# Leo-Liao-Chao/Uncertainty-Aware-CILQR-for-Trajectory-Optimization

Measured on AMD Instinct MI355X. Metric: CILQR solves/sec (N=50, batch B), higher is better.
Workload: dtype f64

## Files before the change

### uncertainty-aware-cilqr-for-trajectory-optimization_amd/csrc/cilqr_api.cpp

```cpp
#include <math.h>
#include <stdarg.h>
#include <stdio.h>
#include <stdlib.h>
#include <string.h>

#include <new>
#include <string>

#include "cilqr_internal.h"

#include "cilqr_handle.h"

namespace cilqr {
thread_local std::string g_last_error;

int fail(int code, const char* fmt, ...) {
  char buf[512];
  va_list ap;
  va_start(ap, fmt);
  vsnprintf(buf, sizeof(buf), fmt, ap);
  va_end(ap);
  g_last_error = buf;
  return code;
}
// ... 166 lines not shown

  cilqr_handle* h = new (std::nothrow) cilqr_handle();
  if (!h) return fail(CILQR_ERR_ARG, "out of host memory");
  memset(h, 0, sizeof(*h));
  h->params = *p;
  derive(*p, h->kp);
  h->device = device;
  h->simds = prop.multiProcessorCount > 0 ? prop.multiProcessorCount * 4 : 1024;
  h->max_batch = max_batch; h->max_horizon = max_horizon; h->max_obstacles = max_obstacles;
  if (const char* fg = getenv("CILQR_FORCE_G")) h->force_g = atoi(fg);
  const size_t B = max_batch, N = max_horizon, M = max_obstacles;
  hipError_t err = hipStreamCreateWithFlags(&h->stream, hipStreamNonBlocking);
  {
    const cilqr::IoLayout plain = cilqr::io_layout(B, N, M, true, 0), sampled = cilqr::io_layout(B, N, M, false, 1);
    h->arena_cap = plain.end > sampled.end ? plain.end : sampled.end;
    if (err == hipSuccess) err = hipMalloc((void**)&h->d_arena, h->arena_cap);
    h->stage_cap = h->arena_cap < ((size_t)1 << 20) ? h->arena_cap : ((size_t)1 << 20);
    if (err == hipSuccess) err = hipHostMalloc((void**)&h->stage, h->stage_cap, hipHostMallocDefault);
  }
  const size_t Bpad = (B + 63) / 64 * 64;
  if (err == hipSuccess) err = dmalloc(&h->d_obs_tab, Bpad * M * N * 6);
  if (err == hipSuccess) err = dmalloc(&h->d_ws, cilqr::solve_groups_ws_doubles(max_batch, max_horizon));
  if (err == hipSuccess) err = dmalloc(&h->d_redo, B);
  if (err == hipSuccess) err = dmalloc(&h->d_hint_passes, B);
  if (err == hipSuccess) err = dmalloc(&h->d_order, B);
  h->hint_B = 0; h->hint_stream = nullptr;
  h->hint_off = getenv("CILQR_NO_SCHEDULE_HINT") != nullptr;
  h->pair_on = getenv("CILQR_PAIR_KERNEL") != nullptr;
  h->steal_off = getenv("CILQR_NO_LANE_SHARING") != nullptr;
  h->split_off = getenv("CILQR_NO_SPLIT_KERNEL") != nullptr;
  h->share_off = getenv("CILQR_NO_SHARE_KERNEL") != nullptr;
  if (const char* kb = getenv("CILQR_LDS_TABLE_KB")) h->tab_budget_kb = atoi(kb);
  h->share_max = -1;
  if (const char* sw = getenv("CILQR_SHARE_W")) h->share_w = atoi(sw) == 3 ? 3 : 2;
  if (const char* sm = getenv("CILQR_SHARE_MAX_B")) h->share_max = atoi(sm);
  if (const char* sw = getenv("CILQR_SPLIT_W")) h->split_w = atoi(sw);
  if (err == hipSuccess) err = dmalloc(&h->d_pair, (size_t)2);
  if (err == hipSuccess) err = dmalloc(&h->d_triple, (size_t)3);
  if (err == hipSuccess) err = dmalloc(&h->d_gather, (size_t)3);
  h->comm_ranks = 1;
  if (err == hipSuccess) err = dmalloc(&h->d_oob, (size_t)1);
  if (err == hipSuccess) err = dmalloc(&h->d_poses, (size_t)8 * 1024 * 4);
  if (err == hipSuccess) err = dmalloc(&h->d_occ_steps, (size_t)8 * 128);
  if (err == hipSuccess) {
    void* unused = nullptr;
    const size_t W = (size_t)p->num_of_local_wpts;
    if (cilqr::scratch_bytes(h, cilqr::SCR_PLAN_IO, (B * (4 + CILQR_POLY_COEFFS + 2 + 2 * W)) * sizeof(double) + B * sizeof(int32_t), &unused) != CILQR_OK ||
        cilqr::scratch_bytes(h, cilqr::SCR_PLAN_PATH, 2 * 1024 * sizeof(double), &unused) != CILQR_OK)
      err = hipErrorOutOfMemory;
  }
  if (err != hipSuccess) {
    int rc = fail(CILQR_ERR_HIP, "cilqr_create: device allocation failed: %s", hipGetErrorString(err));
    cilqr_destroy(h);
    return rc;
  }
  *out = h;
  return CILQR_OK;
}

int cilqr_destroy(cilqr_handle* h) {
  if (!h) return CILQR_OK;
  (void)hipSetDevice(h->device);
  if (h->stream) (void)hipStreamSynchronize(h->stream);
  (void)cilqr_comm_destroy(h);
  if (h->stage) (void)hipHostFree(h->stage);
  for (void* p : h->scratch)
    if (p) (void)hipFree(p);
  void* ptrs[] = {h->d_poses, h->d_unc_layer, h->d_triple, h->d_gather, h->d_arena, h->d_obs_tab, h->d_ws, h->d_redo, h->d_hint_passes, h->d_order, h->d_pair, h->d_src, h->d_dst, h->d_bbox, h->d_oob, h->d_occ_steps};
  for (void* p : ptrs)
    if (p) (void)hipFree(p);
  if (h->stream) (void)hipStreamDestroy(h->stream);
  delete h;
  return CILQR_OK;
}

int cilqr_set_diag_buffer(cilqr_handle* h, uint64_t* dev_buf) {
  if (!h) return fail(CILQR_ERR_ARG, "null handle");
  h->diag = (unsigned long long*)dev_buf;
  return CILQR_OK;
}

namespace {
int fill_unc(const cilqr_handle* h, const cilqr_uncertainty_map* m, cilqr::UncArgs& u) {
  if (!m || !m->layer) return fail(CILQR_ERR_ARG, "cilqr_set_uncertainty_map: null map or layer");
  const cilqr_map_geom& g = m->geom;
  if (g.rows < 2 || g.cols < 2 || !(g.res > 0.0) || !(g.len_x > 0.0) || !(g.len_y > 0.0))
    return fail(CILQR_ERR_ARG, "cilqr_set_uncertainty_map: bad geometry (needs at least 2x2 cells)");
  if (m->probes_l < 1 || m->probes_w < 1 || m->probes_l > 64 || m->probes_w > 64)
    return fail(CILQR_ERR_ARG, "cilqr_set_uncertainty_map: probes_l / probes_w must be in [1, 64]");
  if (m->layer_stride < 0 || (m->layer_stride > 0 && m->layer_stride < (int64_t)g.rows * g.cols))
    return fail(CILQR_ERR_ARG, "cilqr_set_uncertainty_map: layer_stride smaller than one layer");
// ... 146 lines not shown
  const int w = pick_split_wavefronts(h, B);
  if (w < 2 || N > 64 || n_obs < w) return 1;
  return w >= 4 ? 4 : 2;
}

int cilqr_solve_batch_device(cilqr_handle* h, void* stream, int B, int N, int M, const double* x0, double* U,
                             const double* poly, const double* xplan_fl, const double* obs_pose, const double* obs_dim,
                             const double* obs_weight, double* X_out, double* J_out, int32_t* iters_out,
                             int32_t* status_out, uint32_t flags) {
  int rc = check_sizes(h, B, N, M);
  if (rc) return rc;
  if (B == 0) return CILQR_OK;
  if (!x0 || !U || !poly || !xplan_fl || !X_out) return fail(CILQR_ERR_ARG, "cilqr_solve_batch: null required pointer");
  if (M > 0 && (!obs_pose || !obs_dim)) return fail(CILQR_ERR_ARG, "cilqr_solve_batch: M > 0 but obstacle tables are null");
  cilqr::SolveArgs a;
  a.x0 = x0; a.U = U; a.poly = poly; a.xplan_fl = xplan_fl;
  a.obs_pose = obs_pose; a.obs_dim = obs_dim; a.obs_weight = M > 0 ? obs_weight : nullptr;
  a.X_out = X_out; a.J_out = J_out; a.iters_out = iters_out; a.status_out = status_out;
  a.samp_off = nullptr; a.n_samples = 0; a.samp_w = 0.0;
  a.obs_tab = h->d_obs_tab;
  a.fwd = h->d_ws;
  a.order = nullptr; a.hint_passes = nullptr; a.pair = 0; a.tab_budget = 0; a.steal = h->steal_off ? 0 : 1; a.split = 0;
  a.redo = h->d_redo;
  a.diag = h->diag;
  a.passes = h->passes;
  a.unc = h->unc;
  a.B = B; a.N = N; a.M = M; a.flags = flags;
  a.kp = h->kp;
  HIP_TRY(hipSetDevice(h->device));
  const int G = pick_group_lanes(h, B, N, M);
  if (G == 64 && cilqr::solve_lds_bytes(N, h->kp.n_samples) > cilqr::SOLVE_LDS_MAX)
    return fail(CILQR_ERR_UNSUPPORTED, "cilqr_solve_batch: horizon %d needs %zu bytes of LDS per solve (limit %zu)", N,
                cilqr::solve_lds_bytes(N, h->kp.n_samples), cilqr::SOLVE_LDS_MAX);
  if (G == 64) return launch_wave_scheduled(h, a, stream);
  HIP_TRY(cilqr::launch_solve_groups(a, G, h->d_ws, (hipStream_t)stream));
  return CILQR_OK;
}

}

extern "C" {

int cilqr_solve_batch(cilqr_handle* h, int B, int N, int M, const double* x0, double* U, const double* poly,
                      const double* xplan_fl, const double* obs_pose, const double* obs_dim, const double* obs_weight,
                      double* X_out, double* J_out, int32_t* iters_out, int32_t* status_out, uint32_t flags) {
  int rc = check_sizes(h, B, N, M);
// ... 12 lines not shown
                                     const double* nom_dim, const double* sample_offset, double sample_weight, double* X_out,
                                     double* J_out, int32_t* iters_out, int32_t* status_out, uint32_t flags) {
  if (n_obs < 1 || n_samples < 2) return fail(CILQR_ERR_ARG, "cilqr_solve_batch_sampled: needs n_obs >= 1 and n_samples >= 2");
  if ((long)n_obs * n_samples > 1 << 20) return fail(CILQR_ERR_ARG, "cilqr_solve_batch_sampled: n_obs * n_samples too large");
  int rc = check_sizes(h, B, N, n_obs * n_samples);
  if (rc) return rc;
  if (B == 0) return CILQR_OK;
  if (!x0 || !U || !poly || !xplan_fl || !X_out || !nom_pose || !nom_dim || !sample_offset)
    return fail(CILQR_ERR_ARG, "cilqr_solve_batch_sampled: null required pointer");
  if (cilqr::solve_lds_bytes(N, h->kp.n_samples) + cilqr::solve_sampled_lds_bytes(n_obs, n_samples) > cilqr::SOLVE_LDS_MAX)
    return fail(CILQR_ERR_UNSUPPORTED, "cilqr_solve_batch_sampled: n_obs * n_samples offset records do not fit LDS beside the solve");
  if (cilqr::solve_sampled_tab_doubles(n_obs, N) > (size_t)h->max_obstacles * 6 * (size_t)h->max_horizon)
    return fail(CILQR_ERR_UNSUPPORTED, "cilqr_solve_batch_sampled: nominal records exceed the obstacle workspace reserved at create");
  cilqr::SolveArgs a;
  a.x0 = x0; a.U = U; a.poly = poly; a.xplan_fl = xplan_fl;
  a.obs_pose = nom_pose; a.obs_dim = nom_dim; a.obs_weight = nullptr;
  a.X_out = X_out; a.J_out = J_out; a.iters_out = iters_out; a.status_out = status_out;
  a.samp_off = sample_offset; a.n_samples = n_samples; a.samp_w = sample_weight;
  a.obs_tab = h->d_obs_tab;
  a.fwd = h->d_ws;
  a.pair = 0; a.tab_budget = 0; a.steal = 0;
  a.split = pick_split_wavefronts(h, B);
  a.redo = h->d_redo;
  a.diag = h->diag;
  a.passes = h->passes;
  a.unc = h->unc;
  a.B = B; a.N = N; a.M = n_obs; a.flags = flags;
  a.kp = h->kp;
  HIP_TRY(hipSetDevice(h->device));
  return launch_wave_scheduled(h, a, stream);
}

int cilqr_solve_batch_sampled(cilqr_handle* h, int B, int N, int n_obs, int n_samples, const double* x0, double* U,
                              const double* poly, const double* xplan_fl, const double* nom_pose, const double* nom_dim,
                              const double* sample_offset, double sample_weight, double* X_out, double* J_out,
                              int32_t* iters_out, int32_t* status_out, uint32_t flags) {
  if (n_obs < 1 || n_samples < 2) return fail(CILQR_ERR_ARG, "cilqr_solve_batch_sampled: needs n_obs >= 1 and n_samples >= 2");
  if ((long)n_obs * n_samples > 1 << 20) return fail(CILQR_ERR_ARG, "cilqr_solve_batch_sampled: n_obs * n_samples too large");
  int rc = check_sizes(h, B, N, n_obs * n_samples);
  if (rc) return rc;
  if (B == 0) return CILQR_OK;
  if (!x0 || !U || !poly || !xplan_fl || !X_out || !nom_pose || !nom_dim || !sample_offset)
    return fail(CILQR_ERR_ARG, "cilqr_solve_batch_sampled: null required pointer");
  cilqr::HostBatch q{B, N, n_obs, n_samples, x0, U, poly, xplan_fl, nom_pose, nom_dim, nullptr, sample_offset, sample_weight, X_out, J_out,
                     iters_out, status_out, flags};
  rc = cilqr::host_solve_enqueue(h, q);
// ... 287 lines not shown
```

### uncertainty-aware-cilqr-for-trajectory-optimization_amd/csrc/cilqr_handle.h

```cpp
#pragma once

#include <string>

#include "cilqr_internal.h"

struct ncclComm;

struct cilqr_handle;

namespace cilqr {
struct IoLayout {
  size_t x0, poly, xplan, obs_w, samp_off, obs_pose, obs_dim, U, X, J, iters, status, end;
};
IoLayout io_layout(size_t B, size_t N, size_t M, bool weights, size_t n_samples);
struct HostBatch {
  int B, N, M, n_samples;
  const double *x0;
  double* U;
  const double *poly, *xplan_fl, *obs_pose, *obs_dim, *obs_weight, *samp_off;
  double samp_w;
  double *X_out, *J_out;
  int32_t *iters_out, *status_out;
  uint32_t flags;
};
// ... 16 lines not shown
    hipError_t e_ = (expr);                                                                                \
    if (e_ != hipSuccess) return cilqr::fail(CILQR_ERR_HIP, "%s failed: %s", #expr, hipGetErrorString(e_)); \
  } while (0)

struct cilqr_handle {
  cilqr_params params;
  cilqr::KParams kp;
  int device;
  int simds;
  int max_batch, max_horizon, max_obstacles;
  hipStream_t stream;
  char* d_arena;
  size_t arena_cap;
  char* stage;
  size_t stage_cap;
  cilqr::PendingOut pending;
  int debug_fail_enqueue;
  double* d_J;
  void* scratch[cilqr::SCR_SLOTS];
  size_t scratch_cap[cilqr::SCR_SLOTS];
  double* d_obs_tab;
  double* d_ws;
  int32_t* d_redo;
  int32_t* d_hint_passes;
  int32_t* d_order;
  int hint_B;
  void* hint_stream;
  int hint_off;
  int steal_off;
  int split_w;
  int split_off;
  int share_off;
  int tab_budget_kb;
  int share_w;
  int share_max;
  int pair_on;
  int force_g;
  double* d_pair;
  float *d_src, *d_dst, *d_bbox;
  size_t src_cap, dst_cap, bbox_cap;
  unsigned long long* d_oob;
  double* d_poses;
  unsigned pose_slot;
  float* d_occ_steps;
  unsigned occ_slot;
  unsigned long long* diag;
// ... 10 lines not shown
```

### uncertainty-aware-cilqr-for-trajectory-optimization_amd/csrc/cilqr_internal.h

```cpp
#pragma once

#include <hip/hip_runtime.h>
#include <stdint.h>

#include "cilqr.h"

namespace cilqr {

struct KParams {
  double dt;
  double desired_speed;
  double tolerance;
  double w_acc, w_yawrate, w_pos, w_vel, w_obstacle;
  double q1_acc, q2_acc, q1_yawrate, q2_yawrate;
  double q1_front, q2_front, q1_rear, q2_rear;
  double acc_max, acc_min;
  double yaw_hi, yaw_lo;
  double half_dt2;
  double wheelbase, speed_max;
  double t_safe, s_safe_a, s_safe_b, ego_rad, ego_front, ego_rear;
  double lamb_factor, lamb_max;
  int32_t max_iterations;
  int32_t n_samples;
};
// ... 9 lines not shown
  double q1, q2, scale;
};

constexpr int DIAG_SLOTS = 16;

struct SolveArgs {
  const double* x0;
  double* U;
  const double* poly;
  const double* xplan_fl;
  const double* obs_pose;
  const double* obs_dim;
  const double* obs_weight;
  double* X_out;
  double* J_out;
  int32_t* iters_out;
  int32_t* status_out;
  const double* samp_off;
  int32_t n_samples;
  double samp_w;
  double* obs_tab;
  double* fwd;
  int32_t* redo;
  unsigned long long* diag;
  int32_t* passes;
  const int32_t* order;
  int32_t* hint_passes;
  int32_t B, N, M;
  uint32_t flags;
  int32_t pair;
  int32_t tab_budget;
  int32_t steal;
  int32_t split;
  KParams kp;
  UncArgs unc;
};

hipError_t launch_solve_wave(const SolveArgs& a, hipStream_t stream);
hipError_t launch_schedule_order(const int32_t* passes, int B, int32_t* order, hipStream_t stream);
size_t solve_lds_bytes(int N, int n_samples);
constexpr size_t SOLVE_LDS_MAX = 160 * 1024;
bool solve_table_in_lds(int N, int M, int n_samples, int budget);
bool solve_share_applies(int N, int M, int n_samples, int budget);
size_t solve_sampled_lds_bytes(int n_obs, int n_samples);
size_t solve_sampled_tab_doubles(int n_obs, int N);
hipError_t launch_solve_groups(const SolveArgs& a, int G, double* ws, hipStream_t stream);
// ... 60 lines not shown
```

### uncertainty-aware-cilqr-for-trajectory-optimization_amd/csrc/cilqr_select.hip

```cpp
#include "cilqr_internal.h"

namespace cilqr {

namespace {

constexpr int AM_THREADS = 1024;

__device__ __forceinline__ void amin_merge(double& j0, long long& i0, double j1, long long i1) {
  if (j1 < j0 || (j1 == j0 && i1 < i0)) { j0 = j1; i0 = i1; }
}

__global__ __launch_bounds__(AM_THREADS) void argmin_kernel(const double* J, int B, double* out_pair, double* out_triple, double offset,
                                                            double pair_offset) {
  __shared__ double sj[AM_THREADS / 64];
  __shared__ long long si[AM_THREADS / 64];
  constexpr long long NONE = 0x7fffffffffffffffll;
  double bj = __builtin_huge_val();
  long long bi = NONE;
  for (int i = threadIdx.x; i < B; i += AM_THREADS) amin_merge(bj, bi, J[i], i);
  for (int o = 32; o > 0; o >>= 1) {
    const double oj = __shfl_xor(bj, o, 64);
    const long long oi = __shfl_xor(bi, o, 64);
    amin_merge(bj, bi, oj, oi);
  }
  const int lane = threadIdx.x & 63, wave = threadIdx.x >> 6;
  if (lane == 0) { sj[wave] = bj; si[wave] = bi; }
  __syncthreads();
  if (threadIdx.x == 0) {
    for (int w = 1; w < AM_THREADS / 64; ++w) amin_merge(bj, bi, sj[w], si[w]);
    const double idx = (bi == NONE) ? -1.0 : (double)bi;
    if (out_pair) { out_pair[0] = bj; out_pair[1] = idx < 0.0 ? idx : idx + pair_offset; }
    if (out_triple) { out_triple[0] = bj; out_triple[1] = idx; out_triple[2] = offset; }
  }
}

__global__ __launch_bounds__(64) void select_kernel(const double* triples, int n_ranks, double* out_pair) {
  constexpr long long NONE = 0x7fffffffffffffffll;
  double bj = __builtin_huge_val();
  long long bi = NONE;
  for (int r = threadIdx.x; r < n_ranks; r += 64) {
    const double j = triples[3 * r], idx = triples[3 * r + 1], off = triples[3 * r + 2];
    if (idx >= 0.0) amin_merge(bj, bi, j, (long long)idx + (long long)off);
  }
  for (int o = 32; o > 0; o >>= 1) {
    const double oj = __shfl_xor(bj, o, 64);
    const long long oi = __shfl_xor(bi, o, 64);
    amin_merge(bj, bi, oj, oi);
  }
  if (threadIdx.x == 0) {
    out_pair[0] = bj;
    out_pair[1] = (bi == NONE) ? -1.0 : (double)bi;
  }
}

}

hipError_t launch_argmin(const double* J, int B, double* out_pair, double* out_triple, double offset, hipStream_t stream,
                         double pair_offset) {
  hipLaunchKernelGGL(argmin_kernel, dim3(1), dim3(AM_THREADS), 0, stream, J, B, out_pair, out_triple, offset, pair_offset);
  return hipGetLastError();
}

hipError_t launch_select(const double* triples, int n_ranks, double* out_pair, hipStream_t stream) {
  hipLaunchKernelGGL(select_kernel, dim3(1), dim3(64), 0, stream, triples, n_ranks, out_pair);
  return hipGetLastError();
}

}
```

### uncertainty-aware-cilqr-for-trajectory-optimization_amd/csrc/cilqr_solve.hip

```cpp
#include "cilqr_device.hpp"

namespace cilqr {

using namespace dev;

namespace {

constexpr int RECF = REC - 2;
constexpr int FREC = 16;

__device__ __forceinline__ double readfirstlane_f64(double v) {
  int lo = __double2loint(v), hi = __double2hiint(v);
  lo = __builtin_amdgcn_readfirstlane(lo);
  hi = __builtin_amdgcn_readfirstlane(hi);
  return __hiloint2double(hi, lo);
}

__device__ __forceinline__ double wave_sum(double v) {
#pragma unroll
  for (int o = 32; o > 0; o >>= 1) v += __shfl_xor(v, o, WAVE);
  return v;
}

template <int CTRL>
// ... 613 lines not shown
__device__ __forceinline__ bool rollout_fast(const KParams& kp, int N, const double* x0, const double* U, double* X) {
  FwdConst k;
  make_fwd_const(k, kp);
  State s;
  s.x = x0[0]; s.y = x0[1]; s.v = x0[2]; s.th = x0[3];
  const bool th0_ok = fabs(s.th) < MAX_HEADING0;
  double max_turn = 0.0;
  sincos_loop(s.th, s.s, s.c);
  store_state(X, 0, s);
  for (int i = 0; i < N; ++i) {
    dyn_step_loop(k, s, U[2 * i], U[2 * i + 1], max_turn);
    if (PUBLISH) {
      double* r = X + (i + 1) * XR;
      r[0] = s.x; r[1] = s.y; r[4] = s.c; r[5] = s.s;
      asm volatile("" ::: "memory");
      r[2] = s.v; r[3] = s.th;
    } else {
      store_state(X, i + 1, s);
    }
  }
  return th0_ok && max_turn <= MAX_TURN;
}

template <bool DIAG, int TAB, bool GENERAL, bool UNC>
__global__ __launch_bounds__(WAVE, UNC ? 1 : 2) void cilqr_solve_kernel(SolveArgs a) {
  unsigned long long tk0 = 0, tk = 0, c_pro = 0, c_L = 0, c_R = 0, c_F = 0, n_L = 0, n_R = 0;
  unsigned long long sub[8] = {0, 0, 0, 0, 0, 0, 0, 0};
  if (DIAG) tk0 = tk = __builtin_readcyclecounter();
#define CILQR_STAMP(acc)                                 \
  if (DIAG) {                                            \
    const unsigned long long now_ = __builtin_readcyclecounter(); \
    acc += now_ - tk;                                    \
    tk = now_;                                           \
  }
  extern __shared__ __attribute__((aligned(16))) double lds[];
  if ((int)blockIdx.x >= a.B) return;
  const int b = __builtin_amdgcn_readfirstlane(a.order ? a.order[blockIdx.x] : (int)blockIdx.x);
  const int lane = threadIdx.x;
  const KParams kp = a.kp;
  const int N = a.N, M = a.M, S = kp.n_samples;
  const int n_entries = TAB == 2 ? M * a.n_samples : M;
  const bool has_unc = UNC;
  if (b >= a.B) return;
  if (GENERAL && a.redo[b] == 0) return;

  constexpr int RECW = GENERAL ? REC : RECF;
  constexpr bool FSMEM = !GENERAL && TAB == 1;
  const bool twin = GENERAL || (a.flags & CILQR_FLAG_FAITHFUL_ITERS) != 0;
  double* samp = lds;
  double* Xa = samp + ((S + 1) & ~1);
  double* Xb = twin ? Xa + (N + 1) * XR : Xa;
  double* Ua = Xb + (N + 1) * XR;
  double* Ub = twin ? Ua + 2 * N : Ua;
  double* rec = Ub + 2 * N;
  double* kK = rec;
  double* cst = rec + N * RECW;
  double* fwd = a.fwd + (size_t)b * (N + 1) * FREC;
  double* tab = TAB == 1 ? cst + RCST : a.obs_tab + (size_t)b * M * (TAB == 2 ? NOMF : TABF) * N;
  double* off = cst + RCST;
  double* rmax = off + (size_t)M * a.n_samples * OFFF;

  SampleGrid grid;
  make_sample_grid(grid, a.xplan_fl[2 * b], a.xplan_fl[2 * b + 1], S);
  {
    const double* pc = a.poly + (size_t)b * CILQR_POLY_COEFFS;
    for (int s = lane; s < S; s += WAVE) {
      double xs;
// ... 95 lines not shown
    if (GENERAL) {
      forward_general(kp, N, Xc, Uc, kK, Xn, Un);
    } else if (!(FSMEM ? forward_smem(KParams(phase_params()), N, Xc, fwd, Xn, Un) : forward_fast<RECW>(KParams(phase_params()), N, Xc, Uc, kK, Xn, Un))) {
      handover = true;
      break;
    }
    __syncthreads();
    CILQR_STAMP(c_F)
    if (accept) {
      double* t0 = Xc; Xc = Xn; Xn = t0;
      double* t1 = Uc; Uc = Un; Un = t1;
      j_valid = false;
      lamb = lamb / kp.lamb_factor;
      if (fabs(J_new - J_old) < kp.tolerance) { status = CILQR_EXIT_TOLERANCE; break; }
    } else {
      lamb = lamb * kp.lamb_factor;
      if (lamb > kp.lamb_max) { status = CILQR_EXIT_LAMBDA_MAX; break; }
    }
    J_old = J_new;
  }

  if (!GENERAL) {
    int32_t* const hint = phase_args().hint_passes;
    if (lane == 0) {
      phase_args().redo[b] = handover ? 1 : 0;
      if (handover && hint) hint[b] = 63;
    }
    if (handover) return;
  }

  __syncthreads();
  const SolveArgs ae = phase_args();
  double* Uo = ae.U + (size_t)b * 2 * N;
  for (int i = lane; i < 2 * N; i += WAVE) Uo[i] = Uc[i];
  double* Xg = ae.X_out + (size_t)b * 4 * (N + 1);
  for (int i = lane; i < 4 * (N + 1); i += WAVE) Xg[i] = Xc[(i >> 2) * XR + (i & 3)];
  if (ae.J_out) {
    if (!j_valid) J_new = wave_sum_uniform(cost_only(ae.kp, N, lane, samp, S, grid, Xc, Uc));
    if (lane == 0) ae.J_out[b] = J_new;
  }
  if (lane == 0) {
    if (ae.iters_out) ae.iters_out[b] = iters;
    if (ae.status_out) ae.status_out[b] = status;
    if (ae.passes) ae.passes[b] = n_pass;
    if (ae.hint_passes && !GENERAL) ae.hint_passes[b] = n_pass;
  }
  if (DIAG && lane == 0 && a.diag) {
    const unsigned long long now_ = __builtin_readcyclecounter();
    unsigned long long* o = a.diag + (size_t)b * DIAG_SLOTS;
    o[0] = c_pro; o[1] = c_L; o[2] = c_R; o[3] = c_F; o[4] = now_ - tk; o[5] = n_L; o[6] = n_R; o[7] = now_ - tk0;
    for (int q = 0; q < 8; ++q) o[8 + q] = sub[q];
  }
#undef CILQR_STAMP
}

constexpr unsigned long long THETA_PENDING = 0x7FF00000DEADBEEFull;
constexpr int PAIR_CTL = 4;
constexpr int PAIR_SPIN = 1 << 16;
constexpr int CMD_GO = 1, CMD_EXIT = 2;
constexpr int PAIR_LAST = 10;

template <int K>
__device__ __forceinline__ double quad_bcast(double v) {
  return dpp_f64<K * 0x55>(v);
}
template <int K>
__device__ __forceinline__ int quad_bcast_i(int v) { return __builtin_amdgcn_update_dpp(v, v, K * 0x55, 0xF, 0xF, false); }

template <bool LONG_NAP>
__device__ __forceinline__ bool state_arrived(const double* X, int k, int& budget) {
  const volatile unsigned long long* p = reinterpret_cast<const volatile unsigned long long*>(X + k * XR + 3);
  while (*p == THETA_PENDING) {
    if (--budget < 0) return false;
    if (LONG_NAP) __builtin_amdgcn_s_sleep(16); else __builtin_amdgcn_s_sleep(1);
  }
  asm volatile("" ::: "memory");
// ... 234 lines not shown
    __syncthreads();
    CILQR_STAMP(c_R)
    ++n_pass;
    if (DIAG) ++n_R;
    const bool f_ok = forward_smem<true>(KParams(phase_params()), N, Xa, fwd, Xa, Ua);
    CILQR_STAMP(c_F)
    if (dbg) __syncthreads();
    __syncthreads();
    CILQR_STAMP(c_L)
    if (!f_ok) { handover = true; break; }
    lamb = lamb / kp.lamb_factor;
    if (fabs(J_new - J_old) < kp.tolerance) {
      status = CILQR_EXIT_TOLERANCE;
      J_new = *reinterpret_cast<volatile double*>(ctl);
      break;
    }
    J_old = J_new;
    if (it + 1 >= max_it) J_new = *reinterpret_cast<volatile double*>(ctl);
  }
  if (lane == 0) *reinterpret_cast<volatile int*>(cmd) = CMD_EXIT;
  __syncthreads();

  int32_t* const hint = phase_args().hint_passes;
  if (lane == 0) {
    phase_args().redo[b] = handover ? 1 : 0;
    if (handover && hint) hint[b] = 63;
  }
  if (handover) return;

  const SolveArgs ae = phase_args();
  double* Uo = ae.U + (size_t)b * 2 * N;
  for (int i = lane; i < 2 * N; i += WAVE) Uo[i] = Ua[i];
  double* Xg = ae.X_out + (size_t)b * 4 * (N + 1);
  for (int i = lane; i < 4 * (N + 1); i += WAVE) Xg[i] = Xa[(i >> 2) * XR + (i & 3)];
  if (lane == 0) {
    if (ae.J_out) ae.J_out[b] = J_new;
    if (ae.iters_out) ae.iters_out[b] = iters;
    if (ae.status_out) ae.status_out[b] = status;
    if (ae.passes) ae.passes[b] = n_pass;
    if (ae.hint_passes) ae.hint_passes[b] = n_pass;
  }
  if (DIAG && lane == 0 && a.diag) {
    const unsigned long long now_ = __builtin_readcyclecounter();
    unsigned long long* o = a.diag + (size_t)b * DIAG_SLOTS;
    o[0] = c_pro; o[1] = c_L; o[2] = c_R; o[3] = c_F; o[4] = now_ - tk; o[5] = n_L; o[6] = n_R; o[7] = now_ - tk0;
    for (int q = 4; q < 8; ++q) o[8 + q] = sub[q];
  }
#undef CILQR_STAMP
}
// ... 155 lines not shown
      } else {
        CILQR_STAMP(c_R)
        ++n_pass;
        if (DIAG) ++n_R;
        if (!forward_fast<RECF>(KParams(phase_params()), N, Xa, Ua, rec, Xa, Ua)) {
          handover = true;
          stop = true;
        } else {
          j_valid = false;
          lamb = lamb / kp.lamb_factor;
          if (fabs(J_new - J_old) < kp.tolerance) { status = CILQR_EXIT_TOLERANCE; stop = true; }
          J_old = J_new;
          if (it + 1 >= max_it) stop = true;
        }
      }
    }
    if (stop && lane == 0) *reinterpret_cast<volatile int*>(cmd) = CMD_EXIT;
    __syncthreads();
    CILQR_STAMP(c_F)
    if (stop) break;
  }

  int32_t* const hint = phase_args().hint_passes;
  if (lane == 0) {
    phase_args().redo[b] = handover ? 1 : 0;
    if (handover && hint) hint[b] = 63;
  }
  if (handover) return;

  const SolveArgs ae = phase_args();
  double* Uo = ae.U + (size_t)b * 2 * N;
  for (int i = lane; i < 2 * N; i += WAVE) Uo[i] = Ua[i];
  double* Xg = ae.X_out + (size_t)b * 4 * (N + 1);
  for (int i = lane; i < 4 * (N + 1); i += WAVE) Xg[i] = Xa[(i >> 2) * XR + (i & 3)];
  if (ae.J_out) {
    if (!j_valid) J_new = wave_sum_uniform(cost_only(ae.kp, N, lane, samp, S, grid, Xa, Ua));
    if (lane == 0) ae.J_out[b] = J_new;
  }
  if (lane == 0) {
    if (ae.iters_out) ae.iters_out[b] = iters;
    if (ae.status_out) ae.status_out[b] = status;
    if (ae.passes) ae.passes[b] = n_pass;
    if (ae.hint_passes) ae.hint_passes[b] = n_pass;
  }
  if (DIAG && lane == 0 && a.diag) {
    const unsigned long long now_ = __builtin_readcyclecounter();
    unsigned long long* o = a.diag + (size_t)b * DIAG_SLOTS;
    o[0] = c_pro; o[1] = c_L; o[2] = c_R; o[3] = c_F; o[4] = now_ - tk; o[5] = n_L; o[6] = n_R; o[7] = now_ - tk0;
    for (int q = 8; q < DIAG_SLOTS; ++q) o[q] = 0;
// ... 248 lines not shown
      } else {
        CILQR_STAMP(c_R)
        ++n_pass;
        if (DIAG) ++n_R;
        if (!forward_smem(KParams(phase_params()), N, Xa, fwd, Xa, Ua)) {
          handover = true;
          stop = true;
        } else {
          j_valid = false;
          lamb = lamb / kp.lamb_factor;
          if (fabs(J_new - J_old) < kp.tolerance) { status = CILQR_EXIT_TOLERANCE; stop = true; }
          J_old = J_new;
          if (it + 1 >= max_it) stop = true;
        }
      }
    }
    if (stop && lane == 0) *reinterpret_cast<volatile int*>(cmd) = CMD_EXIT;
    __syncthreads();
    CILQR_STAMP(c_F)
    if (stop) break;
  }

  int32_t* const hint = phase_args().hint_passes;
  if (lane == 0) {
    phase_args().redo[b] = handover ? 1 : 0;
    if (handover && hint) hint[b] = 63;
  }
  if (handover) return;

  const SolveArgs ae = phase_args();
  double* Uo = ae.U + (size_t)b * 2 * N;
  for (int i = lane; i < 2 * N; i += WAVE) Uo[i] = Ua[i];
  double* Xg = ae.X_out + (size_t)b * 4 * (N + 1);
  for (int i = lane; i < 4 * (N + 1); i += WAVE) Xg[i] = Xa[(i >> 2) * XR + (i & 3)];
  if (ae.J_out) {
    if (!j_valid) J_new = wave_sum_uniform(cost_only(ae.kp, N, lane, samp, S, grid, Xa, Ua));
    if (lane == 0) ae.J_out[b] = J_new;
  }
  if (lane == 0) {
    if (ae.iters_out) ae.iters_out[b] = iters;
    if (ae.status_out) ae.status_out[b] = status;
    if (ae.passes) ae.passes[b] = n_pass;
    if (ae.hint_passes) ae.hint_passes[b] = n_pass;
  }
  if (DIAG && lane == 0 && a.diag) {
    const unsigned long long now_ = __builtin_readcyclecounter();
    unsigned long long* o = a.diag + (size_t)b * DIAG_SLOTS;
    o[0] = c_pro; o[1] = c_L; o[2] = c_R; o[3] = c_F; o[4] = now_ - tk; o[5] = n_L; o[6] = n_R; o[7] = now_ - tk0;
    o[10] = c_wait;
// ... 63 lines not shown
  mx[3 * i] = h00 * inv; mx[3 * i + 1] = h01 * inv; mx[3 * i + 2] = h11 * inv;
}

size_t core_lds_bytes(int N, int n_samples, bool compact) {
  const size_t traj = (size_t)(N + 1) * XR + (size_t)2 * N;
  const size_t doubles = (((size_t)n_samples + 1) & ~(size_t)1) + (compact ? 1 : 2) * traj + (size_t)N * (compact ? RECF : REC) + RCST;
  return doubles * sizeof(double);
}

template <bool DIAG, int TAB, bool UNC>
hipError_t launch_pair_unc(const SolveArgs& a, size_t extra, hipStream_t stream) {
  const bool faithful = (a.flags & CILQR_FLAG_FAITHFUL_ITERS) != 0;
  const size_t lds_fast = core_lds_bytes(a.N, a.kp.n_samples, !faithful) + extra;
  const size_t lds_general = core_lds_bytes(a.N, a.kp.n_samples, false) + extra;
  if (lds_general > 64 * 1024) {
    hipError_t e = hipFuncSetAttribute(reinterpret_cast<const void*>(&cilqr_solve_kernel<DIAG, TAB, false, UNC>),
                                       hipFuncAttributeMaxDynamicSharedMemorySize, (int)lds_general);
    if (e == hipSuccess)
      e = hipFuncSetAttribute(reinterpret_cast<const void*>(&cilqr_solve_kernel<DIAG, TAB, true, UNC>),
                              hipFuncAttributeMaxDynamicSharedMemorySize, (int)lds_general);
    if (e != hipSuccess) return e;
  }
  hipLaunchKernelGGL((cilqr_solve_kernel<DIAG, TAB, false, UNC>), dim3(a.B), dim3(WAVE), lds_fast, stream, a);
  hipLaunchKernelGGL((cilqr_solve_kernel<DIAG, TAB, true, UNC>), dim3(a.B), dim3(WAVE), lds_general, stream, a);
  return hipGetLastError();
}
template <bool DIAG>
hipError_t launch_two_wavefronts(const SolveArgs& a, size_t tab_bytes, hipStream_t stream) {
  const size_t lds_fast = core_lds_bytes(a.N, a.kp.n_samples, true) + tab_bytes + ((((size_t)a.N + 1) & ~(size_t)1) + PAIR_CTL) * sizeof(double);
  const size_t lds_general = core_lds_bytes(a.N, a.kp.n_samples, false) + tab_bytes;
  hipLaunchKernelGGL((cilqr_solve_pair_kernel<DIAG>), dim3(a.B), dim3(2 * WAVE), lds_fast, stream, a);
  hipLaunchKernelGGL((cilqr_solve_kernel<DIAG, 1, true, false>), dim3(a.B), dim3(WAVE), lds_general, stream, a);
  return hipGetLastError();
}
template <int W, bool LONG, bool DIAG, bool UNC>
hipError_t launch_shared_L(const SolveArgs& a, size_t tab_bytes, hipStream_t stream) {
  const size_t lds_fast = core_lds_bytes(a.N, a.kp.n_samples, true) + tab_bytes +
                          ((((size_t)((W - 1) + (UNC ? 1 : 0)) * 5 * a.N + 1) & ~(size_t)1) + 4) * sizeof(double);
  const size_t lds_general = core_lds_bytes(a.N, a.kp.n_samples, false) + tab_bytes;
  if (lds_fast > 64 * 1024 || lds_general > 64 * 1024) {
    const int want = (int)(lds_fast > lds_general ? lds_fast : lds_general);
    hipError_t e = hipFuncSetAttribute(reinterpret_cast<const void*>(&cilqr_solve_share_kernel<W, LONG, DIAG, UNC>), hipFuncAttributeMaxDynamicSharedMemorySize, want);
    if (e == hipSuccess)
      e = hipFuncSetAttribute(reinterpret_cast<const void*>(&cilqr_solve_kernel<DIAG, 1, true, UNC>), hipFuncAttributeMaxDynamicSharedMemorySize, want);
    if (e != hipSuccess) return e;
  }
  hipLaunchKernelGGL((cilqr_solve_share_kernel<W, LONG, DIAG, UNC>), dim3(a.B), dim3(W * WAVE), lds_fast, stream, a);
  hipLaunchKernelGGL((cilqr_solve_kernel<DIAG, 1, true, UNC>), dim3(a.B), dim3(WAVE), lds_general, stream, a);
  return hipGetLastError();
}
template <bool DIAG, bool UNC>
hipError_t launch_shared_L_by_shape(const SolveArgs& a, size_t tab_bytes, hipStream_t stream) {
  if (a.N > WAVE) return launch_shared_L<2, true, DIAG, UNC>(a, tab_bytes, stream);
  if (a.pair == 3 && (UNC || a.M >= 2)) return launch_shared_L<3, false, DIAG, UNC>(a, tab_bytes, stream);
  return launch_shared_L<2, false, DIAG, UNC>(a, tab_bytes, stream);
}
template <bool DIAG, int TAB>
hipError_t launch_pair(const SolveArgs& a, size_t extra, hipStream_t stream) {
  return a.unc.layer ? launch_pair_unc<DIAG, TAB, true>(a, extra, stream) : launch_pair_unc<DIAG, TAB, false>(a, extra, stream);
}

}

size_t solve_lds_bytes(int N, int n_samples) { return core_lds_bytes(N, n_samples, false); }
bool solve_table_in_lds(int N, int M, int n_samples, int budget) {
  return solve_lds_bytes(N, n_samples) + (size_t)M * TABF * N * sizeof(double) <= (size_t)(budget > 0 ? budget : 32 * 1024);
}
bool solve_share_applies(int N, int M, int n_samples, int budget) { return N < 2 * WAVE && solve_table_in_lds(N, M, n_samples, budget); }

size_t solve_sampled_lds_bytes(int n_obs, int n_samples) {
  return ((size_t)n_obs * n_samples * OFFF + (size_t)2 * n_obs) * sizeof(double);
// ... 41 lines not shown

hipError_t launch_quu_inverse(int n, const double* q, const double* lamb, double* out, int general, hipStream_t stream) {
  if (n <= 0) return hipSuccess;
  hipLaunchKernelGGL(quu_inverse_kernel, dim3((n + 63) / 64), dim3(64), 0, stream, n, q, lamb, out, general);
  return hipGetLastError();
}

hipError_t launch_solve_wave(const SolveArgs& a, hipStream_t stream) {
  if (a.B <= 0) return hipSuccess;
  const size_t lds = solve_lds_bytes(a.N, a.kp.n_samples);
  const size_t tab_bytes = (size_t)a.M * TABF * a.N * sizeof(double);
  const bool tab_lds = a.n_samples == 0 && solve_table_in_lds(a.N, a.M, a.kp.n_samples, a.tab_budget);
  if (a.n_samples > 0) {
    const size_t extra = solve_sampled_lds_bytes(a.M, a.n_samples);
    if (lds + extra > SOLVE_LDS_MAX) return hipErrorInvalidValue;
    if (a.split >= 2 && a.N <= WAVE && a.M >= a.split && (a.flags & CILQR_FLAG_FAITHFUL_ITERS) == 0) {
      const int W = a.split >= 4 ? 4 : 2;
      const bool unc = a.unc.layer != nullptr;
      const size_t lds_fast = core_lds_bytes(a.N, a.kp.n_samples, true) + extra + ((((size_t)((W - 1) + (unc ? 1 : 0)) * 5 * a.N + 1) & ~(size_t)1) + 2) * sizeof(double);
      const size_t lds_general = core_lds_bytes(a.N, a.kp.n_samples, false) + extra;
      if (lds_fast <= 64 * 1024 && lds_general <= 64 * 1024) {
#define CILQR_SPLIT_LAUNCH(WW, DD, UU)                                                                                          \
  hipLaunchKernelGGL((cilqr_solve_split_kernel<WW, DD, UU>), dim3(a.B), dim3(WW * WAVE), lds_fast, stream, a);                 \
  hipLaunchKernelGGL((cilqr_solve_kernel<DD, 2, true, UU>), dim3(a.B), dim3(WAVE), lds_general, stream, a);
        if (a.diag) {
          if (unc) { if (W == 4) { CILQR_SPLIT_LAUNCH(4, true, true) } else { CILQR_SPLIT_LAUNCH(2, true, true) } }
          else { if (W == 4) { CILQR_SPLIT_LAUNCH(4, true, false) } else { CILQR_SPLIT_LAUNCH(2, true, false) } }
        } else {
          if (unc) { if (W == 4) { CILQR_SPLIT_LAUNCH(4, false, true) } else { CILQR_SPLIT_LAUNCH(2, false, true) } }
          else { if (W == 4) { CILQR_SPLIT_LAUNCH(4, false, false) } else { CILQR_SPLIT_LAUNCH(2, false, false) } }
        }
#undef CILQR_SPLIT_LAUNCH
        return hipGetLastError();
      }
    }
    return a.diag ? launch_pair<true, 2>(a, extra, stream) : launch_pair<false, 2>(a, extra, stream);
  }
  if (lds > SOLVE_LDS_MAX) return hipErrorInvalidValue;
  const size_t extra = tab_lds ? tab_bytes : 0;
  if (tab_lds && a.pair == 1 && !a.unc.layer && (a.flags & CILQR_FLAG_FAITHFUL_ITERS) == 0)
    return a.diag ? launch_two_wavefronts<true>(a, tab_bytes, stream) : launch_two_wavefronts<false>(a, tab_bytes, stream);
  if (a.pair >= 2 && a.n_samples == 0 && solve_share_applies(a.N, a.M, a.kp.n_samples, a.tab_budget) && (a.flags & CILQR_FLAG_FAITHFUL_ITERS) == 0) {
    if (a.unc.layer) return a.diag ? launch_shared_L_by_shape<true, true>(a, tab_bytes, stream) : launch_shared_L_by_shape<false, true>(a, tab_bytes, stream);
    return a.diag ? launch_shared_L_by_shape<true, false>(a, tab_bytes, stream) : launch_shared_L_by_shape<false, false>(a, tab_bytes, stream);
  }
  if (a.diag) return tab_lds ? launch_pair<true, 1>(a, extra, stream) : launch_pair<true, 0>(a, extra, stream);
  return tab_lds ? launch_pair<false, 1>(a, extra, stream) : launch_pair<false, 0>(a, extra, stream);
// ... 4 lines not shown
```

Measured before the change: 2.441 million.

## Compact handover solves into a work list and shrink follow-up grid

Fast-path kernels now append handed-over solves to an atomic work list instead of writing a per-solve redo flag. The general follow-up kernel launches a smaller grid sized to the device and loops over only the listed solves, resetting the list counters through a last-block atomic. This removes launching one wave per batch element just to exit early. The argmin kernel is also rewritten with DPP and readlane reductions, vectorised double2 loads, and a wave count sized to B. The in-kernel counter reset relies on correct ordering across launches, and the reused list makes concurrent calls on the same handle risky.

```diff
diff --git a/uncertainty-aware-cilqr-for-trajectory-optimization_amd/csrc/cilqr_api.cpp b/uncertainty-aware-cilqr-for-trajectory-optimization_amd/csrc/cilqr_api.cpp
--- a/uncertainty-aware-cilqr-for-trajectory-optimization_amd/csrc/cilqr_api.cpp
+++ b/uncertainty-aware-cilqr-for-trajectory-optimization_amd/csrc/cilqr_api.cpp
@@ -212,6 +212,9 @@
   if (err == hipSuccess) err = dmalloc(&h->d_obs_tab, Bpad * M * N * 6);
   if (err == hipSuccess) err = dmalloc(&h->d_ws, cilqr::solve_groups_ws_doubles(max_batch, max_horizon));
   if (err == hipSuccess) err = dmalloc(&h->d_redo, B);
+  if (err == hipSuccess) err = dmalloc(&h->d_redo_list, 2 + B);
+  if (err == hipSuccess) err = hipMemsetAsync(h->d_redo_list, 0, 2 * sizeof(int32_t), h->stream);
+  if (err == hipSuccess) err = hipStreamSynchronize(h->stream);
   if (err == hipSuccess) err = dmalloc(&h->d_hint_passes, B);
   if (err == hipSuccess) err = dmalloc(&h->d_order, B);
   h->hint_B = 0; h->hint_stream = nullptr;
@@ -256,7 +259,7 @@
   if (h->stage) (void)hipHostFree(h->stage);
   for (void* p : h->scratch)
     if (p) (void)hipFree(p);
-  void* ptrs[] = {h->d_poses, h->d_unc_layer, h->d_triple, h->d_gather, h->d_arena, h->d_obs_tab, h->d_ws, h->d_redo, h->d_hint_passes, h->d_order, h->d_pair, h->d_src, h->d_dst, h->d_bbox, h->d_oob, h->d_occ_steps};
+  void* ptrs[] = {h->d_poses, h->d_unc_layer, h->d_triple, h->d_gather, h->d_arena, h->d_obs_tab, h->d_ws, h->d_redo, h->d_redo_list, h->d_hint_passes, h->d_order, h->d_pair, h->d_src, h->d_dst, h->d_bbox, h->d_oob, h->d_occ_steps};
   for (void* p : ptrs)
     if (p) (void)hipFree(p);
   if (h->stream) (void)hipStreamDestroy(h->stream);
@@ -449,6 +452,8 @@
   a.fwd = h->d_ws;
   a.order = nullptr; a.hint_passes = nullptr; a.pair = 0; a.tab_budget = 0; a.steal = h->steal_off ? 0 : 1; a.split = 0;
   a.redo = h->d_redo;
+  a.redo_list = h->d_redo_list;
+  a.follow_grid = B < h->simds / 4 ? B : h->simds / 4;
   a.diag = h->diag;
   a.passes = h->passes;
   a.unc = h->unc;
@@ -507,6 +512,8 @@
   a.pair = 0; a.tab_budget = 0; a.steal = 0;
   a.split = pick_split_wavefronts(h, B);
   a.redo = h->d_redo;
+  a.redo_list = h->d_redo_list;
+  a.follow_grid = B < h->simds / 4 ? B : h->simds / 4;
   a.diag = h->diag;
   a.passes = h->passes;
   a.unc = h->unc;
diff --git a/uncertainty-aware-cilqr-for-trajectory-optimization_amd/csrc/cilqr_handle.h b/uncertainty-aware-cilqr-for-trajectory-optimization_amd/csrc/cilqr_handle.h
--- a/uncertainty-aware-cilqr-for-trajectory-optimization_amd/csrc/cilqr_handle.h
+++ b/uncertainty-aware-cilqr-for-trajectory-optimization_amd/csrc/cilqr_handle.h
@@ -62,6 +62,7 @@
   double* d_obs_tab;
   double* d_ws;
   int32_t* d_redo;
+  int32_t* d_redo_list;
   int32_t* d_hint_passes;
   int32_t* d_order;
   int hint_B;
diff --git a/uncertainty-aware-cilqr-for-trajectory-optimization_amd/csrc/cilqr_internal.h b/uncertainty-aware-cilqr-for-trajectory-optimization_amd/csrc/cilqr_internal.h
--- a/uncertainty-aware-cilqr-for-trajectory-optimization_amd/csrc/cilqr_internal.h
+++ b/uncertainty-aware-cilqr-for-trajectory-optimization_amd/csrc/cilqr_internal.h
@@ -55,6 +55,8 @@
   double* obs_tab;
   double* fwd;
   int32_t* redo;
+  int32_t* redo_list;
+  int32_t follow_grid;
   unsigned long long* diag;
   int32_t* passes;
   const int32_t* order;
diff --git a/uncertainty-aware-cilqr-for-trajectory-optimization_amd/csrc/cilqr_select.hip b/uncertainty-aware-cilqr-for-trajectory-optimization_amd/csrc/cilqr_select.hip
--- a/uncertainty-aware-cilqr-for-trajectory-optimization_amd/csrc/cilqr_select.hip
+++ b/uncertainty-aware-cilqr-for-trajectory-optimization_amd/csrc/cilqr_select.hip
@@ -4,31 +4,81 @@
 
 namespace {
 
-constexpr int AM_THREADS = 1024;
+constexpr int AM_WAVE = 64;
+constexpr int AM_MAX_WAVES = 16;
+constexpr int AM_LOADS = 8;
+constexpr int AM_PER_WAVE = 4096;
+constexpr int AM_NONE = 0x7fffffff;
 
 __device__ __forceinline__ void amin_merge(double& j0, long long& i0, double j1, long long i1) {
   if (j1 < j0 || (j1 == j0 && i1 < i0)) { j0 = j1; i0 = i1; }
 }
+__device__ __forceinline__ void amin_merge(double& j0, int& i0, double j1, int i1) {
+  if (j1 < j0 || (j1 == j0 && i1 < i0)) { j0 = j1; i0 = i1; }
+}
 
-__global__ __launch_bounds__(AM_THREADS) void argmin_kernel(const double* J, int B, double* out_pair, double* out_triple, double offset,
-                                                            double pair_offset) {
-  __shared__ double sj[AM_THREADS / 64];
-  __shared__ long long si[AM_THREADS / 64];
-  constexpr long long NONE = 0x7fffffffffffffffll;
+template <int CTRL>
+__device__ __forceinline__ void amin_dpp(double& bj, int& bi) {
+  const int lo = __builtin_amdgcn_update_dpp(__double2loint(bj), __double2loint(bj), CTRL, 0xF, 0xF, false);
+  const int hi = __builtin_amdgcn_update_dpp(__double2hiint(bj), __double2hiint(bj), CTRL, 0xF, 0xF, false);
+  const int oi = __builtin_amdgcn_update_dpp(bi, bi, CTRL, 0xF, 0xF, false);
+  amin_merge(bj, bi, __hiloint2double(hi, lo), oi);
+}
+__device__ __forceinline__ void amin_readlane(double& bj, int& bi, double vj, int vi, int l) {
+  const int lo = __builtin_amdgcn_readlane(__double2loint(vj), l);
+  const int hi = __builtin_amdgcn_readlane(__double2hiint(vj), l);
+  amin_merge(bj, bi, __hiloint2double(hi, lo), __builtin_amdgcn_readlane(vi, l));
+}
+__device__ __forceinline__ void amin_wave(double& bj, int& bi) {
+  amin_dpp<0xB1>(bj, bi);
+  amin_dpp<0x4E>(bj, bi);
+  amin_dpp<0x141>(bj, bi);
+  amin_dpp<0x140>(bj, bi);
+  const double vj = bj;
+  const int vi = bi;
+  bj = __builtin_huge_val();
+  bi = AM_NONE;
+  for (int r = 0; r < AM_WAVE; r += 16) amin_readlane(bj, bi, vj, vi, r);
+}
+
+__global__ __launch_bounds__(AM_MAX_WAVES * AM_WAVE) void argmin_kernel(const double* J, int B, double* out_pair, double* out_triple,
+                                                                        double offset, double pair_offset) {
+  __shared__ double sj[AM_MAX_WAVES];
+  __shared__ int si[AM_MAX_WAVES];
+  const int lane = threadIdx.x & (AM_WAVE - 1), wave = threadIdx.x / AM_WAVE, waves = blockDim.x / AM_WAVE;
   double bj = __builtin_huge_val();
-  long long bi = NONE;
-  for (int i = threadIdx.x; i < B; i += AM_THREADS) amin_merge(bj, bi, J[i], i);
-  for (int o = 32; o > 0; o >>= 1) {
-    const double oj = __shfl_xor(bj, o, 64);
-    const long long oi = __shfl_xor(bi, o, 64);
-    amin_merge(bj, bi, oj, oi);
+  int bi = AM_NONE;
+  const double nan = __builtin_nan("");
+  if ((reinterpret_cast<size_t>(J) & 15) == 0) {
+    constexpr int CHUNK = AM_LOADS * 2 * AM_WAVE;
+    for (int base = wave * CHUNK; base < B; base += waves * CHUNK) {
+      double2 v[AM_LOADS];
+#pragma unroll
+      for (int k = 0; k < AM_LOADS; ++k) {
+        const int i = base + 2 * (lane + k * AM_WAVE);
+        v[k] = i + 1 < B ? *reinterpret_cast<const double2*>(J + i) : make_double2(i < B ? J[i] : nan, nan);
+      }
+#pragma unroll
+      for (int k = 0; k < AM_LOADS; ++k) {
+        const int i = base + 2 * (lane + k * AM_WAVE);
+        amin_merge(bj, bi, v[k].x, i);
+        amin_merge(bj, bi, v[k].y, i + 1);
+      }
+    }
+  } else {
+    for (int i = threadIdx.x; i < B; i += blockDim.x) amin_merge(bj, bi, J[i], i);
   }
-  const int lane = threadIdx.x & 63, wave = threadIdx.x >> 6;
-  if (lane == 0) { sj[wave] = bj; si[wave] = bi; }
-  __syncthreads();
+  amin_wave(bj, bi);
+  if (waves > 1) {
+    if (lane == 0) { sj[wave] = bj; si[wave] = bi; }
+    __syncthreads();
+    if (wave != 0) return;
+    bj = lane < waves ? sj[lane] : __builtin_huge_val();
+    bi = lane < waves ? si[lane] : AM_NONE;
+    amin_wave(bj, bi);
+  }
   if (threadIdx.x == 0) {
-    for (int w = 1; w < AM_THREADS / 64; ++w) amin_merge(bj, bi, sj[w], si[w]);
-    const double idx = (bi == NONE) ? -1.0 : (double)bi;
+    const double idx = (bi == AM_NONE) ? -1.0 : (double)bi;
     if (out_pair) { out_pair[0] = bj; out_pair[1] = idx < 0.0 ? idx : idx + pair_offset; }
     if (out_triple) { out_triple[0] = bj; out_triple[1] = idx; out_triple[2] = offset; }
   }
@@ -57,7 +107,8 @@
 
 hipError_t launch_argmin(const double* J, int B, double* out_pair, double* out_triple, double offset, hipStream_t stream,
                          double pair_offset) {
-  hipLaunchKernelGGL(argmin_kernel, dim3(1), dim3(AM_THREADS), 0, stream, J, B, out_pair, out_triple, offset, pair_offset);
+  const int waves = B <= AM_PER_WAVE ? 1 : B >= AM_MAX_WAVES * AM_PER_WAVE ? AM_MAX_WAVES : (B + AM_PER_WAVE - 1) / AM_PER_WAVE;
+  hipLaunchKernelGGL(argmin_kernel, dim3(1), dim3(waves * AM_WAVE), 0, stream, J, B, out_pair, out_triple, offset, pair_offset);
   return hipGetLastError();
 }
 
diff --git a/uncertainty-aware-cilqr-for-trajectory-optimization_amd/csrc/cilqr_solve.hip b/uncertainty-aware-cilqr-for-trajectory-optimization_amd/csrc/cilqr_solve.hip
--- a/uncertainty-aware-cilqr-for-trajectory-optimization_amd/csrc/cilqr_solve.hip
+++ b/uncertainty-aware-cilqr-for-trajectory-optimization_amd/csrc/cilqr_solve.hip
@@ -659,8 +659,13 @@
   return th0_ok && max_turn <= MAX_TURN;
 }
 
+__device__ __forceinline__ void hand_over(int b) {
+  int32_t* const list = phase_args().redo_list;
+  list[2 + atomicAdd(list, 1)] = b;
+}
+
 template <bool DIAG, int TAB, bool GENERAL, bool UNC>
-__global__ __launch_bounds__(WAVE, UNC ? 1 : 2) void cilqr_solve_kernel(SolveArgs a) {
+__device__ __forceinline__ void solve_wave(const SolveArgs& a, const int b) {
   unsigned long long tk0 = 0, tk = 0, c_pro = 0, c_L = 0, c_R = 0, c_F = 0, n_L = 0, n_R = 0;
   unsigned long long sub[8] = {0, 0, 0, 0, 0, 0, 0, 0};
   if (DIAG) tk0 = tk = __builtin_readcyclecounter();
@@ -671,15 +676,11 @@
     tk = now_;                                           \
   }
   extern __shared__ __attribute__((aligned(16))) double lds[];
-  if ((int)blockIdx.x >= a.B) return;
-  const int b = __builtin_amdgcn_readfirstlane(a.order ? a.order[blockIdx.x] : (int)blockIdx.x);
   const int lane = threadIdx.x;
   const KParams kp = a.kp;
   const int N = a.N, M = a.M, S = kp.n_samples;
   const int n_entries = TAB == 2 ? M * a.n_samples : M;
   const bool has_unc = UNC;
-  if (b >= a.B) return;
-  if (GENERAL && a.redo[b] == 0) return;
 
   constexpr int RECW = GENERAL ? REC : RECF;
   constexpr bool FSMEM = !GENERAL && TAB == 1;
@@ -821,9 +822,9 @@
 
   if (!GENERAL) {
     int32_t* const hint = phase_args().hint_passes;
-    if (lane == 0) {
-      phase_args().redo[b] = handover ? 1 : 0;
-      if (handover && hint) hint[b] = 63;
+    if (lane == 0 && handover) {
+      hand_over(b);
+      if (hint) hint[b] = 63;
     }
     if (handover) return;
   }
@@ -851,6 +852,27 @@
     for (int q = 0; q < 8; ++q) o[8 + q] = sub[q];
   }
 #undef CILQR_STAMP
+}
+
+template <bool DIAG, int TAB, bool GENERAL, bool UNC>
+__global__ __launch_bounds__(WAVE, UNC ? 1 : 2) void cilqr_solve_kernel(SolveArgs a) {
+  if (!GENERAL) {
+    if ((int)blockIdx.x >= a.B) return;
+    const int b = __builtin_amdgcn_readfirstlane(a.order ? a.order[blockIdx.x] : (int)blockIdx.x);
+    if (b < a.B) solve_wave<DIAG, TAB, false, UNC>(a, b);
+    return;
+  }
+  int32_t* const list = a.redo_list;
+  const int n = __builtin_amdgcn_readfirstlane(list[0]);
+  if (threadIdx.x == 0 && __hip_atomic_fetch_add(list + 1, 1, __ATOMIC_ACQ_REL, __HIP_MEMORY_SCOPE_AGENT) == (int)gridDim.x - 1) {
+    list[0] = 0;
+    list[1] = 0;
+  }
+  for (int k = blockIdx.x; k < n; k += gridDim.x) {
+    const int b = __builtin_amdgcn_readfirstlane(list[2 + k]);
+    __syncthreads();
+    solve_wave<DIAG, TAB, true, UNC>(a, b);
+  }
 }
 
 constexpr unsigned long long THETA_PENDING = 0x7FF00000DEADBEEFull;
@@ -1131,9 +1153,9 @@
   __syncthreads();
 
   int32_t* const hint = phase_args().hint_passes;
-  if (lane == 0) {
-    phase_args().redo[b] = handover ? 1 : 0;
-    if (handover && hint) hint[b] = 63;
+  if (lane == 0 && handover) {
+    hand_over(b);
+    if (hint) hint[b] = 63;
   }
   if (handover) return;
 
@@ -1335,9 +1357,9 @@
   }
 
   int32_t* const hint = phase_args().hint_passes;
-  if (lane == 0) {
-    phase_args().redo[b] = handover ? 1 : 0;
-    if (handover && hint) hint[b] = 63;
+  if (lane == 0 && handover) {
+    hand_over(b);
+    if (hint) hint[b] = 63;
   }
   if (handover) return;
 
@@ -1632,9 +1654,9 @@
   }
 
   int32_t* const hint = phase_args().hint_passes;
-  if (lane == 0) {
-    phase_args().redo[b] = handover ? 1 : 0;
-    if (handover && hint) hint[b] = 63;
+  if (lane == 0 && handover) {
+    hand_over(b);
+    if (hint) hint[b] = 63;
   }
   if (handover) return;
 
@@ -1744,7 +1766,7 @@
     if (e != hipSuccess) return e;
   }
   hipLaunchKernelGGL((cilqr_solve_kernel<DIAG, TAB, false, UNC>), dim3(a.B), dim3(WAVE), lds_fast, stream, a);
-  hipLaunchKernelGGL((cilqr_solve_kernel<DIAG, TAB, true, UNC>), dim3(a.B), dim3(WAVE), lds_general, stream, a);
+  hipLaunchKernelGGL((cilqr_solve_kernel<DIAG, TAB, true, UNC>), dim3(a.follow_grid), dim3(WAVE), lds_general, stream, a);
   return hipGetLastError();
 }
 template <bool DIAG>
@@ -1752,7 +1774,7 @@
   const size_t lds_fast = core_lds_bytes(a.N, a.kp.n_samples, true) + tab_bytes + ((((size_t)a.N + 1) & ~(size_t)1) + PAIR_CTL) * sizeof(double);
   const size_t lds_general = core_lds_bytes(a.N, a.kp.n_samples, false) + tab_bytes;
   hipLaunchKernelGGL((cilqr_solve_pair_kernel<DIAG>), dim3(a.B), dim3(2 * WAVE), lds_fast, stream, a);
-  hipLaunchKernelGGL((cilqr_solve_kernel<DIAG, 1, true, false>), dim3(a.B), dim3(WAVE), lds_general, stream, a);
+  hipLaunchKernelGGL((cilqr_solve_kernel<DIAG, 1, true, false>), dim3(a.follow_grid), dim3(WAVE), lds_general, stream, a);
   return hipGetLastError();
 }
 template <int W, bool LONG, bool DIAG, bool UNC>
@@ -1768,7 +1790,7 @@
     if (e != hipSuccess) return e;
   }
   hipLaunchKernelGGL((cilqr_solve_share_kernel<W, LONG, DIAG, UNC>), dim3(a.B), dim3(W * WAVE), lds_fast, stream, a);
-  hipLaunchKernelGGL((cilqr_solve_kernel<DIAG, 1, true, UNC>), dim3(a.B), dim3(WAVE), lds_general, stream, a);
+  hipLaunchKernelGGL((cilqr_solve_kernel<DIAG, 1, true, UNC>), dim3(a.follow_grid), dim3(WAVE), lds_general, stream, a);
   return hipGetLastError();
 }
 template <bool DIAG, bool UNC>
@@ -1856,7 +1878,7 @@
       if (lds_fast <= 64 * 1024 && lds_general <= 64 * 1024) {
 #define CILQR_SPLIT_LAUNCH(WW, DD, UU)                                                                                          \
   hipLaunchKernelGGL((cilqr_solve_split_kernel<WW, DD, UU>), dim3(a.B), dim3(WW * WAVE), lds_fast, stream, a);                 \
-  hipLaunchKernelGGL((cilqr_solve_kernel<DD, 2, true, UU>), dim3(a.B), dim3(WAVE), lds_general, stream, a);
+  hipLaunchKernelGGL((cilqr_solve_kernel<DD, 2, true, UU>), dim3(a.follow_grid), dim3(WAVE), lds_general, stream, a);
         if (a.diag) {
           if (unc) { if (W == 4) { CILQR_SPLIT_LAUNCH(4, true, true) } else { CILQR_SPLIT_LAUNCH(2, true, true) } }
           else { if (W == 4) { CILQR_SPLIT_LAUNCH(4, true, false) } else { CILQR_SPLIT_LAUNCH(2, true, false) } }
```

Measured after the change: 2.421 million, median of 2. About the same (-0.8%).
